# xiaolong-li1/VIDEO-BLADE

Measured on AMD Instinct MI355X. Metric: frames/sec (aggregate over n_gpus; per GPU = value/n_gpus), CogVideoX-5B 8-step 49x720x480 bf16 (attention path); attn TFLOPS vs dense, higher is better.
Workload: dtype bf16; 1 GPU; CogVideoX-5B 8-step 49x720x480 bf16: 336 inner_attention calls per video (8 steps x 42 blocks), q/k/v [1,48,17776,64] (13x30x45 latent tokens + 226 text); global_batch=1, seq_len=17776, heads=48, head_dim=64, mask=energy rule (reference defaults), parallelism=replicas x1 (prompt-batch DP, no collective)

## Files before the change

video-blade_amd/csrc/vb_attn_fwd.hip:

```cpp
#include <type_traits>

#include "vb_args.hpp"
#include "vb_attn_fwd.hpp"
#include "vb_trace.hpp"

#ifndef VB_ATTN_TRACE
#define VB_ATTN_TRACE 0
#endif
#if VB_ATTN_TRACE
namespace vb { __device__ TraceBuf g_attn_trace; }
#define VB_ATRACE_START(k) trace_start(g_attn_trace, k, (unsigned)vblk)
#define VB_ATRACE_END() trace_end(g_attn_trace, (unsigned)vblk)
#else
#define VB_ATRACE_START(k)
#define VB_ATRACE_END()
#endif

namespace vb {

#ifndef VB_LAZY_COUNT
#define VB_LAZY_COUNT 0
#endif
#if VB_LAZY_COUNT
__device__ unsigned long long g_vb_stamp[16];
#define VB_LAZY_ADD(slot, n) if (lane == 0) atomicAdd(&g_vb_stamp[slot], n)
#else
#define VB_LAZY_ADD(slot, n)
#endif

template <int D, bool kKvRows>
constexpr int fwd_smem_bytes() {
  return ((D == 64) ? 3 : 2) * 2 * kKT * D * 2 + kMaxBlocks * 2 + 16 + (kKvRows ? 4 * 512 : 0);
}

__device__ __forceinline__ int ballot_rank(unsigned long long bal) {
  return __builtin_amdgcn_mbcnt_hi((unsigned)(bal >> 32), __builtin_amdgcn_mbcnt_lo((unsigned)bal, 0u));
}
__device__ __forceinline__ void build_kept_list(const uint8_t* mrow, bool dense, bool use_main, int nbk, int qblk,
                                                int lane, uint16_t* list, int* list_n) {
  int n = 0;
  int dpos = -1;
  if (use_main) {
    for (int j0 = 0; j0 < nbk; j0 += 64) {
      const int j = j0 + lane;
      const bool keep = (j < nbk) && (dense || mrow[j] != 0);
      const unsigned long long bal = __ballot(keep);
      if (keep) {
        const int pos = n + ballot_rank(bal);
        list[pos] = (uint16_t)j;
        if (j == qblk) dpos = pos;
      }
      n += __popcll(bal);
    }
    const unsigned long long db = __ballot(dpos > 0);
    if (db != 0 && qblk != nbk - 1) {
      const int dp = __builtin_amdgcn_readlane(dpos, (int)__builtin_ctzll(db));
      if (lane == 0) {
        const uint16_t t = list[0];
        list[0] = (uint16_t)qblk;
        list[dp] = t;
      }
    }
  }
  if (lane == 0) *list_n = n;
}

__device__ __forceinline__ float half_max(const f32x16& x) {
  const float a = max3f(max3f(max3f(x[0], x[1], x[2]), x[3], x[4]), x[5], x[6]);
  const float c = max3f(max3f(max3f(x[8], x[9], x[10]), x[11], x[12]), x[13], x[14]);
  return max3f(a, c, fmaxf(x[7], x[15]));
}
template <class T, int kPrio>
__device__ __forceinline__ float exp_pack(const f32x16& x, typename T::vec8& p0, typename T::vec8& p1) {
  float e[16];
  float h4[4];
  if constexpr (kPrio & 4) __builtin_amdgcn_s_setprio(1);
#pragma unroll
  for (int r = 0; r < 16; ++r) {
    e[r] = exp2_fast(x[r]);
    h4[r & 3] = r < 4 ? e[r] : h4[r & 3] + e[r];
  }
  u32x4 u0, u1;
#pragma unroll
  for (int w = 0; w < 4; ++w) {
    u0[w] = pack2<T>(e[2 * w], e[2 * w + 1]);
    u1[w] = pack2<T>(e[8 + 2 * w], e[8 + 2 * w + 1]);
  }
  p0 = __builtin_bit_cast(typename T::vec8, u0);
  p1 = __builtin_bit_cast(typename T::vec8, u1);
  if constexpr (kPrio & 4) __builtin_amdgcn_s_setprio(0);
  return (h4[0] + h4[1]) + (h4[2] + h4[3]);
}


template <int D, class T, bool kPool, bool kKvRows, bool kML, bool kCBias, bool kWQ>
__device__ __forceinline__ void attn_fwd_item(const FwdParams& p, const int vblk, int& next) {
  constexpr int KS = D / 16;
  constexpr int DT = D / 32;
  constexpr bool kSplitPV = fwd::split_pv(D);
  constexpr int kPrio = !kCBias ? 0 : D == 64 ? fwd::kPrio64 : fwd::kPrio128;
  constexpr float kLazyBound = std::is_same<T, BF16>::value ? kLazyBoundBF16 : kLazyBoundF16;
  constexpr int kRowB = D * 2;
  constexpr int kMatBytes = kKT * kRowB;
  constexpr int kBufBytes = 2 * kMatBytes;
  constexpr int kBufs = (D == 64) ? 3 : 2;
  constexpr int kChunks = kRowB / 16;
  constexpr int kRowsPerInst = 1024 / kRowB;
  constexpr int kInstPerMat = kMatBytes / 1024;
  constexpr int kInstPerWave = 2 * kInstPerMat / 4;
  __shared__ __attribute__((aligned(16))) uint8_t smem[fwd_smem_bytes<D, kKvRows>()];
  static_assert(fwd_smem_bytes<D, kKvRows>() == kBufs * kBufBytes + kMaxBlocks * 2 + 16 + (kKvRows ? 4 * 512 : 0), "LDS layout");
  static_assert(!(kML && (kPool || kKvRows)), "multi-level mode reads the KV pyramids only");
  uint16_t* list = reinterpret_cast<uint16_t*>(smem + kBufs * kBufBytes);
  int* list_n = reinterpret_cast<int*>(smem + kBufs * kBufBytes + kMaxBlocks * 2);

  int tid = threadIdx.x;
  if constexpr (kWQ) {
    asm volatile("" : "+v"(tid));
    tid &= kThreads - 1;
  }
  const int lane = tid & 63;
  const int wave = __builtin_amdgcn_readfirstlane(tid >> 6);

  const int half = lane >> 5;
  const int l32 = lane & 31;

  VB_ATRACE_START(0);
  int qblk, bh;
  fwd_item_decode(p, vblk, bh, qblk);
  const int b = bh / p.H, h = bh % p.H;

  int Lq = p.Lq, Lk = p.Lk;
  int64_t qrow0 = 0, krow0 = 0;
  if (p.cu_q) {
    qrow0 = p.cu_q[b];
    Lq = p.cu_q[b + 1] - p.cu_q[b];
    krow0 = p.cu_k[b];
    Lk = p.cu_k[b + 1] - p.cu_k[b];
  }
  const int q0 = qblk * kQBlk;
  if (q0 >= Lq) return;
  const int nbk = (Lk + kQBlk - 1) / kQBlk;

  const uint8_t* mrow = nullptr;
  bool dense = true;
  bool nan_head = false;
  if (p.use_main) {
    const uint8_t* mh = head_mask_base(p.mask, p.ms, p.head_mask_type, p.H, b, h, nan_head, p.hm_mode);
    if (mh) {
      dense = false;
      mrow = mh + (int64_t)qblk * p.ms[2];
    }
  }
  if (kML) {
    if (tid < 64) {
      int cnt[4] = {0, 0, 0, 0};
      for (int j0 = 0; j0 < nbk; j0 += 64) {
        const int j = j0 + lane;
        const int lv = j < nbk ? mrow[j] : 0;
#pragma unroll
        for (int e = 0; e < 4; ++e) cnt[e] += __popcll(__ballot(lv == (1 << e)));
      }
      int pos[4] = {0, cnt[0], cnt[0] + cnt[1], cnt[0] + cnt[1] + cnt[2]};
      for (int j0 = 0; j0 < nbk; j0 += 64) {
        const int j = j0 + lane;
        const int lv = j < nbk ? mrow[j] : 0;
#pragma unroll
        for (int e = 0; e < 4; ++e) {
          const unsigned long long bal = __ballot(lv == (1 << e));
          if (lv == (1 << e))
            list[pos[e] + __builtin_amdgcn_mbcnt_hi((unsigned)(bal >> 32),
                                                    __builtin_amdgcn_mbcnt_lo((unsigned)bal, 0u))] = (uint16_t)j;
          pos[e] += __popcll(bal);
        }
      }
      if (lane < 4) list_n[lane] = cnt[0] * (lane == 0) + cnt[1] * (lane == 1) + cnt[2] * (lane == 2) + cnt[3] * (lane == 3);
    }
  } else if (tid < 64) {
    build_kept_list(mrow, dense, p.use_main, nbk, qblk, lane, list, list_n);
  }

  const int qg = q0 + wave * 32 + l32;
  const bool qvalid = qg < Lq;
  int qrow = qvalid ? qg : Lq - 1;
  if (p.q_rows) qrow = p.q_rows[qrow];
  const uint8_t* qbase = reinterpret_cast<const uint8_t*>(p.q) + 2 * (b * p.qs[0] + h * p.qs[1] + qrow0 * p.qs[2]);
  typename T::vec8 qf[KS];
  auto load_q = [&]() __attribute__((always_inline)) {
    const uint8_t* qp = qbase + (int64_t)qrow * 2 * p.qs[2];
#pragma unroll
    for (int s = 0; s < KS; ++s)
      qf[s] = *reinterpret_cast<const typename T::vec8*>(qp + (16 * s + 8 * half) * 2);
    if constexpr (kCBias) {
#pragma unroll
      for (int s = 0; s < KS; ++s)
#pragma unroll
        for (int e = 0; e < 8; ++e) qf[s][e] = T::from_f32(T::to_f32(qf[s][e]) * p.c);
    }
#pragma unroll
    for (int s = 0; s < KS; ++s) asm volatile("" : "+v"(qf[s]));
  };
  constexpr bool kQLate = D == 64 ? fwd::kQLate64 : (kCBias && !kKvRows) ? fwd::kQLate128Lazy : fwd::kQLate128;
  if constexpr (kQLate) {
    asm volatile("s_waitcnt lgkmcnt(0)" ::: "memory");
    __builtin_amdgcn_s_barrier();
    asm volatile("" ::: "memory");
  } else {
    load_q();
    __syncthreads();
  }
  const int nkept = __builtin_amdgcn_readfirstlane(*list_n);
  int ntm = 2 * nkept;
  if (nkept > 0 && list[nkept - 1] == nbk - 1 && (nbk - 1) * kQBlk + kKT >= Lk && !(kML && p.ref_tail)) ntm -= 1;
  const int ntp = kPool ? (p.Lkp + kKT - 1) / kKT : 0;
  int n2 = 0, n4 = 0, n8 = 0, T12 = 0, T124 = 0;
  if (kML) {
    n2 = __builtin_amdgcn_readfirstlane(list_n[1]);
    n4 = __builtin_amdgcn_readfirstlane(list_n[2]);
    n8 = __builtin_amdgcn_readfirstlane(list_n[3]);
    T12 = ntm + n2;
    T124 = T12 + (n4 + 1) / 2;
  }
  const int ntiles = kML ? T124 + (n8 + 3) / 4 : ntm + ntp;

  const uint8_t* kbase = reinterpret_cast<const uint8_t*>(p.k) + 2 * (b * p.ks[0] + h * p.ks[1] + krow0 * p.ks[2]);
  const uint8_t* vbase = reinterpret_cast<const uint8_t*>(p.v) + 2 * (b * p.vs[0] + h * p.vs[1] + krow0 * p.vs[2]);
  const uint8_t* kpbase = nullptr;
  const uint8_t* vpbase = nullptr;
  if (kPool) {
    kpbase = reinterpret_cast<const uint8_t*>(p.kp) + 2 * (b * p.kps[0] + h * p.kps[1]);
    vpbase = reinterpret_cast<const uint8_t*>(p.vp) + 2 * (b * p.vps[0] + h * p.vps[1]);
  }

  auto tile_src = [&](int t, int blk_raw) __attribute__((always_inline)) -> TileSrc {
    TileSrc s;
    if (t < ntm) {
      const int blk = __builtin_amdgcn_readfirstlane(blk_raw);
      s.pooled = 0;
      s.kstart = blk * kQBlk + (t & 1) * kKT;
      s.klen = min(kKT, Lk - s.kstart);
    } else {
      s.pooled = 1;
      s.kstart = (t - ntm) * kKT;
      s.klen = min(kKT, p.Lkp - s.kstart);
    }
    return s;
  };

  const int off4 = p.Lpad + p.Lpad / 2, off8 = off4 + p.Lpad / 4;
  const int my_half = (wave & 1) * 32;
  auto ml_tile_src = [&](int t, int raw) __attribute__((always_inline)) -> MlTileSrc {
    MlTileSrc s;
    const int a = __builtin_amdgcn_readfirstlane(raw & 0xFFFF);
    const int c = __builtin_amdgcn_readfirstlane(raw >> 16);
    if (t < ntm) {
      const int kstart = a * kQBlk + (t & 1) * kKT;
      s.srcA = kstart + my_half;
      s.klen = p.ref_tail ? kKT : min(kKT, Lk - kstart);
      s.lvl = 0;
    } else if (t < T12) {
      s.srcA = p.Lpad + a * 64 + my_half;
      s.klen = kKT;
      s.lvl = 1;
    } else if (t < T124) {
      s.srcA = off4 + a * 32;
      s.klen = min(kKT, (n4 - 2 * (t - T12)) * 32);
      s.lvl = 2;
    } else {
      s.srcA = off8 + a * 16;
      s.klen = min(kKT, (n8 - 4 * (t - T124)) * 16);
      s.lvl = 3;
    }
    s.srcB = (t >= T124) ? off8 + c * 16 : s.srcA + 16;
    return s;
  };
  auto ml_list_at = [&](int t) __attribute__((always_inline)) -> int {
    int e0, e1;
    if (t < ntm) {
      e0 = e1 = t >> 1;
    } else if (t < T12) {
      e0 = e1 = nkept + (t - ntm);
    } else if (t < T124) {
      e0 = e1 = nkept + n2 + min(2 * (t - T12) + (wave & 1), n4 - 1);
    } else {
      const int e = 4 * (t - T124) + 2 * (wave & 1);
      e0 = nkept + n2 + n4 + min(e, n8 - 1);
      e1 = nkept + n2 + n4 + min(e + 1, n8 - 1);
    }
    e0 = min(max(e0, 0), kMaxBlocks - 1);
    e1 = min(max(e1, 0), kMaxBlocks - 1);
    return (int)list[e0] | ((int)list[e1] << 16);
  };

  static_assert(2 * kInstPerWave == kInstPerMat, "DMA split assumes two waves per matrix");
  const int my_mat = wave >> 1;
  const uint8_t* my_base = my_mat == 0 ? kbase : vbase;
  const int64_t my_stride = 2 * (my_mat == 0 ? p.ks[2] : p.vs[2]);
  const uint8_t* my_pbase = my_mat == 0 ? kpbase : vpbase;
  const int64_t my_pstride = kPool ? 2 * (my_mat == 0 ? p.kps[2] : p.vps[2]) : 0;
  int my_chunk[kInstPerWave];
  int my_row[kInstPerWave];
#pragma unroll
  for (int i = 0; i < kInstPerWave; ++i) {
    const int mi = (wave & 1) * kInstPerWave + i;
    const int r = mi * kRowsPerInst + lane / kChunks;
    const int sl = lane % kChunks;
    my_row[i] = r;
    if (my_mat == 0) {
      my_chunk[i] = sl ^ ((D == 64) ? ((r >> 1) & 7) : (r & 15));
    } else {
      const int vsw = (D == 64) ? ((r >> 1) & 1) : (r & 3);
      my_chunk[i] = (((sl >> 2) ^ vsw) << 2) | (sl & 3);
    }
  }
  const int my_rowb = (int)my_stride;
  const int my_prowb = (int)my_pstride;
  const int src_rows = kML ? 15 * (p.Lpad / 8) : Lk;
  const srd_t my_rsrc = make_srd(my_base, p.use_main ? (int)((int64_t)(src_rows - 1) * my_stride + kRowB) : 0);
  const srd_t my_prsrc = make_srd(kPool ? my_pbase : my_base, kPool ? (int)((int64_t)(p.Lkp - 1) * my_pstride + kRowB) : 0);
  int my_voff[kInstPerWave];
  int my_rc[kInstPerWave];
  const int my_row0 = my_row[0];
#pragma unroll
  for (int i = 0; i < kInstPerWave; ++i) {
    my_rc[i] = my_chunk[i] * 16;
    if constexpr (kML) my_voff[i] = (my_row[i] & 15) * my_rowb + my_chunk[i] * 16;
  }
  auto ml_issue = [&](const MlTileSrc src, int slot) __attribute__((always_inline)) {
    uint8_t* dst = smem + slot * kBufBytes + my_mat * kMatBytes + (wave & 1) * kInstPerWave * 1024;
    const int soffA = __builtin_amdgcn_readfirstlane(src.srcA * my_rowb);
    const int soffB = __builtin_amdgcn_readfirstlane(src.srcB * my_rowb);
#pragma unroll
    for (int i = 0; i < kInstPerWave; ++i)
      if constexpr (kWQ) dma16_unscoped(my_rsrc, dst + i * 1024, my_voff[i], (i * kRowsPerInst >= 16) ? soffB : soffA);
      else dma16(my_rsrc, dst + i * 1024, my_voff[i], (i * kRowsPerInst >= 16) ? soffB : soffA);
  };
  const int gather_key = ((wave & 1) * kInstPerWave + (lane % kInstPerWave)) * kRowsPerInst + lane / kInstPerWave;
  const srd_t rows_srd = make_srd(kKvRows ? p.kv_rows : nullptr, kKvRows ? Lk * 4 : 0);
  uint8_t* const ibase = smem + kBufs * kBufBytes + kMaxBlocks * 2 + 16 + wave * 128;
  auto issue_idx = [&](int t, int blk_raw) __attribute__((always_inline)) {
    int voff = 0;
    if (t < ntm) {
      const int kstart = __builtin_amdgcn_readfirstlane(blk_raw) * kQBlk + (t & 1) * kKT;
      voff = 4 * (kstart + min(gather_key, min(kKT, Lk - kstart) - 1));
    }
    if (lane < 32) {
      uint8_t* dst = ibase + (t & 3) * 512;
      if constexpr (kWQ) {
        uint32_t a = __builtin_amdgcn_readfirstlane(
            static_cast<uint32_t>(reinterpret_cast<uintptr_t>((__attribute__((address_space(3))) uint8_t*)dst)));
        asm("" : "+s"(a));
        dst = (uint8_t*)(__attribute__((address_space(3))) uint8_t*)(uintptr_t)a;
      }
      __builtin_amdgcn_raw_ptr_buffer_load_lds(
          __builtin_amdgcn_make_buffer_rsrc(const_cast<void*>(rows_srd.base), (short)0, rows_srd.bytes, 0x00020000),
          (__attribute__((address_space(3))) void*)dst, 4, voff, 0, 0, 0);
    }
  };
  auto issue = [&](const TileSrc src, int slot, int t = 0) __attribute__((always_inline)) {
    uint8_t* dst = smem + slot * kBufBytes + my_mat * kMatBytes + (wave & 1) * kInstPerWave * 1024;
    auto piece = [&](int i, srd_t sd, int voff, int soff) __attribute__((always_inline)) {
      if constexpr (kWQ) dma16_unscoped(sd, dst + i * 1024, voff, soff);
      else dma16(sd, dst + i * 1024, voff, soff);
    };
    const bool pooled = kPool && src.pooled;
    if (kKvRows && !pooled) {
      typedef int i32x4 __attribute__((ext_vector_type(4)));
      int o[kInstPerWave];
      const uint8_t* ib = ibase + (t & 3) * 512 + 4 * kInstPerWave * (lane / kChunks);
#pragma unroll
      for (int c = 0; c < kInstPerWave; c += 4) {
        const i32x4 w = *reinterpret_cast<const i32x4*>(ib + 4 * c);
#pragma unroll
        for (int e = 0; e < 4; ++e) o[c + e] = w[e];
      }
#pragma unroll
      for (int i = 0; i < kInstPerWave; ++i) {
        int voff;
        asm("v_mad_u32_u24 %0, %1, %2, %3" : "=v"(voff) : "v"(o[i]), "s"(my_rowb), "v"(my_chunk[i] * 16));
        piece(i, my_rsrc, voff, 0);
      }
      return;
    }
    const int rowb = pooled ? my_prowb : my_rowb;
    const int soff = __builtin_amdgcn_readfirstlane(src.kstart * rowb);
    if (src.klen == kKT) {
      const int vb0 = (int)__umul24((unsigned)my_row0, (unsigned)rowb);
#pragma unroll
      for (int i = 0; i < kInstPerWave; ++i)
        piece(i, pooled ? my_prsrc : my_rsrc, vb0 + my_rc[i], __builtin_amdgcn_readfirstlane(soff + i * kRowsPerInst * rowb));
    } else {
#pragma unroll
      for (int i = 0; i < kInstPerWave; ++i) {
        const int r = min(my_row0 + i * kRowsPerInst, src.klen - 1);
        piece(i, pooled ? my_prsrc : my_rsrc, r * rowb + my_rc[i], soff);
      }
    }
  };

  f32x16 o[DT];
#pragma unroll
  for (int i = 0; i < DT; ++i)
#pragma unroll
    for (int r = 0; r < 16; ++r) o[i][r] = 0.f;
  float m = kCBias ? 0.f : -INFINITY;
  float l = 0.f;
  f32x16 cb;
#pragma unroll
  for (int r = 0; r < 16; ++r) cb[r] = 0.f;
  int cur_bias_bits = 0;
  bool first = true;

  const int vrow = 4 * half + (lane & 15) / 4;
  const int vcol = 16 * ((lane >> 4) & 1) + 4 * (lane & 3);

  int k_lane[KS];
#pragma unroll
  for (int ks = 0; ks < KS; ++ks) k_lane[ks] = k_off<D>(l32, 2 * ks + half);
  uint32_t v_lane[DT];
#pragma unroll
  for (int dt = 0; dt < DT; ++dt)
    v_lane[dt] = static_cast<uint32_t>(reinterpret_cast<uintptr_t>(
                     (__attribute__((address_space(3))) const uint8_t*)smem)) +
                 v_off_bytes<D>(vrow, dt * 32 + vcol);

  auto tile_step = [&](auto U, int bias_bits, int klen) __attribute__((always_inline)) {
    constexpr int kSlot = decltype(U)::value;
    const uint8_t* kl = smem + kSlot * kBufBytes;
    const float bias = __int_as_float(bias_bits);
    f32x16 s[2];
    constexpr int VPRE = D == 64 ? (kKvRows ? fwd::kVPre64Rows : fwd::kVPre64) : 2;
    s16x4 vlo[4][DT], vhi[4][DT];
    auto read_v = [&](int kk) __attribute__((always_inline)) {
      const int row0 = (kk >> 1) * 32 + 16 * (kk & 1);
#pragma unroll
      for (int dt = 0; dt < DT; ++dt) {
        vlo[kk][dt] = lds_tr4_asm(v_lane[dt], kSlot * kBufBytes + kMatBytes + row0 * kRowB);
        vhi[kk][dt] = lds_tr4_asm(v_lane[dt], kSlot * kBufBytes + kMatBytes + (row0 + 8) * kRowB);
      }
    };
    auto wait_v = [&](int kk) __attribute__((always_inline)) {
#pragma unroll
      for (int dt = 0; dt < DT; ++dt)
        asm volatile("s_waitcnt lgkmcnt(0)" : "+v"(vlo[kk][dt]), "+v"(vhi[kk][dt]));
    };
    auto next_v = [&](int kk) __attribute__((always_inline)) {
      wait_v(kk);
      if (kk + VPRE < 4) read_v(kk + VPRE);
    };
    auto pv = [&](int kk, const typename T::vec8& pf) __attribute__((always_inline)) {
      if constexpr (kPrio & 2) __builtin_amdgcn_s_setprio(1);
#pragma unroll
      for (int dt = 0; dt < DT; ++dt) o[dt] = T::mfma32(join8<T>(vlo[kk][dt], vhi[kk][dt]), pf, o[dt]);
      if constexpr (kPrio & 2) __builtin_amdgcn_s_setprio(0);
    };
    auto mask_tail = [&](int kt) __attribute__((always_inline)) {
#pragma unroll
      for (int r = 0; r < 16; ++r)
        if (kt * 32 + (r & 3) + 8 * (r >> 2) + 4 * half >= klen) s[kt][r] = -INFINITY;
    };
    auto scores = [&](const f32x16& seed) __attribute__((always_inline)) {
      if constexpr (kPrio & 1) __builtin_amdgcn_s_setprio(1);
#pragma unroll
      for (int kt = 0; kt < 2; ++kt) {
        typename T::vec8 kf[KS];
#pragma unroll
        for (int ks = 0; ks < KS; ++ks) kf[ks] = lds_b128<T>(kl + kt * 32 * kRowB, k_lane[ks]);
        s[kt] = T::mfma32(kf[0], qf[0], seed);
#pragma unroll
        for (int ks = 1; ks < KS; ++ks) s[kt] = T::mfma32(kf[ks], qf[ks], s[kt]);
      }
      if constexpr (kPrio & 1) __builtin_amdgcn_s_setprio(0);
    };

    if constexpr (kCBias) {
      if (bias_bits != cur_bias_bits) {
        asm volatile("");
        const float db = bias - __int_as_float(cur_bias_bits);
#pragma unroll
        for (int r = 0; r < 16; ++r) cb[r] += db;
        cur_bias_bits = bias_bits;
      }
      auto raise_m = [&](float mt, auto KT0) __attribute__((always_inline)) {
        constexpr int kt0 = decltype(KT0)::value;
        const float delta = fmaxf(max_xor32(mt), 0.f);
        const float alpha = exp2_fast(-delta);
        m += delta;
        l *= alpha;
#pragma unroll
        for (int i = 0; i < DT; ++i)
#pragma unroll
          for (int r = 0; r < 16; ++r) o[i][r] *= alpha;
#pragma unroll
        for (int r = 0; r < 16; ++r) {
          cb[r] -= delta;
          if (kt0 == 0) s[0][r] -= delta;
          s[1][r] -= delta;
        }
      };
      scores(cb);
#pragma unroll
      for (int kk = 0; kk < VPRE; ++kk) read_v(kk);
      if (klen < kKT) {
        asm volatile("");
        mask_tail(0);
        mask_tail(1);
      }
      if (first) {
        asm volatile("");
        const float mt = max_xor32(fmaxf(half_max(s[0]), half_max(s[1])));
        m += mt;
#pragma unroll
        for (int r = 0; r < 16; ++r) {
          s[0][r] -= mt;
          s[1][r] -= mt;
          cb[r] -= mt;
        }
        first = false;
      }
      typename T::vec8 pf[4];
      if constexpr (kSplitPV) {
#pragma unroll
        for (int kt = 0; kt < 2; ++kt) {
          float hs = exp_pack<T, kPrio>(s[kt], pf[2 * kt], pf[2 * kt + 1]);
          if (!__all(hs <= kLazyBound)) {
            asm volatile("");
            VB_LAZY_ADD(10, 1ull);
            if (kt == 0) raise_m(half_max(s[0]), std::integral_constant<int, 0>{});
            else raise_m(half_max(s[1]), std::integral_constant<int, 1>{});
            hs = exp_pack<T, kPrio>(s[kt], pf[2 * kt], pf[2 * kt + 1]);
          }
          l += hs;
#pragma unroll
          for (int kk = 2 * kt; kk < 2 * kt + 2; ++kk) {
            next_v(kk);
            pv(kk, pf[kk]);
          }
        }
      } else {
        float h0 = exp_pack<T, kPrio>(s[0], pf[0], pf[1]);
        float h1 = exp_pack<T, kPrio>(s[1], pf[2], pf[3]);
        if (!__all(fmaxf(h0, h1) <= kLazyBound)) {
          asm volatile("");
          VB_LAZY_ADD(10, 1ull);
          raise_m(fmaxf(half_max(s[0]), half_max(s[1])), std::integral_constant<int, 0>{});
          h0 = exp_pack<T, kPrio>(s[0], pf[0], pf[1]);
          h1 = exp_pack<T, kPrio>(s[1], pf[2], pf[3]);
        }
        l += h0 + h1;
#pragma unroll
        for (int kk = 0; kk < 4; ++kk) {
          next_v(kk);
          pv(kk, pf[kk]);
        }
      }
      VB_LAZY_ADD(11, kSplitPV ? 2ull : 1ull);
    }

    if constexpr (!kCBias) {
      f32x16 zero;
#pragma unroll
      for (int r = 0; r < 16; ++r) zero[r] = 0.f;
      scores(zero);
#pragma unroll
      for (int kk = 0; kk < VPRE; ++kk) read_v(kk);
      if (klen < kKT) {
        asm volatile("");
#pragma unroll
        for (int kt = 0; kt < 2; ++kt)
#pragma unroll
          for (int r = 0; r < 16; ++r)
            if (kt * 32 + (r & 3) + 8 * (r >> 2) + 4 * half >= klen) s[kt][r] = -INFINITY;
      }
      float mq[4];
#pragma unroll
      for (int c = 0; c < 4; ++c) {
        const f32x16& x = s[c >> 1];
        const int o = 8 * (c & 1);
        mq[c] = max3f(max3f(max3f(x[o], x[o + 1], x[o + 2]), x[o + 3], x[o + 4]), x[o + 5], x[o + 6]);
      }
      const float f1 = max3f(mq[0], mq[1], s[0][7]);
      const float f2 = max3f(mq[2], mq[3], s[0][15]);
      float mt = max3f(max3f(f1, f2, s[1][7]), s[1][15], s[1][15]);
      mt = max_xor32(mt) * p.c + bias;
      if (!__all(mt <= m + fwd::kRescaleSlack)) {
        asm volatile("");
        const float mn = fmaxf(m, mt);
        const float alpha = exp2_fast(m - mn);
        m = mn;
        l *= alpha;
#pragma unroll
        for (int i = 0; i < DT; ++i)
#pragma unroll
          for (int r = 0; r < 16; ++r) o[i][r] *= alpha;
      }
      const float nbias = bias - m;
      float lq[4] = {0.f, 0.f, 0.f, 0.f};
      if constexpr (kSplitPV) {
#pragma unroll
        for (int kt = 0; kt < 2; ++kt) {
#pragma unroll
          for (int r = 0; r < 16; ++r) {
            const float e = exp2_fast(fmaf(s[kt][r], p.c, nbias));
            s[kt][r] = e;
            lq[(2 * kt + r) & 3] = (kt == 0 && r < 4) ? e : lq[(2 * kt + r) & 3] + e;
          }
#pragma unroll
          for (int kk = 2 * kt; kk < 2 * kt + 2; ++kk) {
            wait_v(kk);
            if (kk + VPRE < 4) read_v(kk + VPRE);
            const typename T::vec8 pf = pack8<T>(s[kk >> 1], 8 * (kk & 1));
#pragma unroll
            for (int dt = 0; dt < DT; ++dt) o[dt] = T::mfma32(join8<T>(vlo[kk][dt], vhi[kk][dt]), pf, o[dt]);
          }
        }
        l += (lq[0] + lq[1]) + (lq[2] + lq[3]);
      } else {
#pragma unroll
        for (int kt = 0; kt < 2; ++kt)
#pragma unroll
          for (int r = 0; r < 16; ++r) {
            const float e = exp2_fast(fmaf(s[kt][r], p.c, nbias));
            s[kt][r] = e;
            lq[(2 * kt + r) & 3] = (kt == 0 && r < 4) ? e : lq[(2 * kt + r) & 3] + e;
          }
        l += (lq[0] + lq[1]) + (lq[2] + lq[3]);
#pragma unroll
        for (int kk = 0; kk < 4; ++kk) {
          wait_v(kk);
          if (kk + VPRE < 4) read_v(kk + VPRE);
          const typename T::vec8 pf = pack8<T>(s[kk >> 1], 8 * (kk & 1));
#pragma unroll
          for (int dt = 0; dt < DT; ++dt) o[dt] = T::mfma32(join8<T>(vlo[kk][dt], vhi[kk][dt]), pf, o[dt]);
        }
      }
    }
  };

  auto list_at = [&](int t) __attribute__((always_inline)) -> int {
    return t < ntm ? (int)list[min(t >> 1, kMaxBlocks - 1)] : 0;
  };
  using Src = std::conditional_t<kML, MlTileSrc, TileSrc>;
  auto any_list_at = [&](int t) __attribute__((always_inline)) -> int {
    if constexpr (kML) return ml_list_at(t);
    else return list_at(t);
  };
  auto any_tile_src = [&](int t, int raw) __attribute__((always_inline)) -> Src {
    if constexpr (kML) return ml_tile_src(t, raw);
    else return tile_src(t, raw);
  };
  auto any_issue = [&](const Src src, int slot) __attribute__((always_inline)) {
    if constexpr (kML) ml_issue(src, slot);
    else issue(src, slot);
  };
  Src slot_src[kBufs];
  const int pool_bias_bits = __builtin_amdgcn_readfirstlane(__float_as_int(p.pool_bias_l2));
  int next_blk, idx_blk = 0;
  if constexpr (kKvRows) {
#pragma unroll
    for (int s0 = 0; s0 < kBufs; ++s0) issue_idx(s0, list_at(s0));
    slot_src[0] = tile_src(0, list_at(0));
    VB_WAIT_VMCNT(kBufs - 1);
    asm volatile("" ::: "memory");
    issue(slot_src[0], 0, 0);
    if constexpr (kBufs > 2) {
      slot_src[1] = tile_src(1, list_at(1));
      VB_WAIT_VMCNT(kBufs - 2 + kInstPerWave);
      asm volatile("" ::: "memory");
      issue(slot_src[1], 1, 1);
    }
    next_blk = list_at(kBufs - 1);
    idx_blk = list_at(kBufs);
  } else {
    slot_src[0] = any_tile_src(0, any_list_at(0));
    if (ntiles > 0) any_issue(slot_src[0], 0);
    if constexpr (kBufs > 2) {
      slot_src[1] = any_tile_src(1, any_list_at(1));
      if (ntiles > 1) any_issue(slot_src[1], 1);
    }
    next_blk = any_list_at(kBufs - 1);
  }
  if constexpr (kQLate) load_q();
  auto body = [&](int t, auto U) __attribute__((always_inline)) {
    constexpr int u = decltype(U)::value;
    constexpr int un = (u + kBufs - 1) % kBufs;
    const int ti = t + kBufs - 1;
    if constexpr (kKvRows) {
      if constexpr (kBufs == 3) VB_WAIT_VMCNT(kInstPerWave);
      else VB_WAIT_VMCNT(0);
      asm volatile("s_waitcnt lgkmcnt(0)" ::: "memory");
      __builtin_amdgcn_s_barrier();
      asm volatile("" ::: "memory");
      issue_idx(t + kBufs, idx_blk);
      slot_src[un] = tile_src(ti, next_blk);
      issue(slot_src[un], un, ti);
      next_blk = idx_blk;
      idx_blk = list_at(t + kBufs + 1);
    } else {
      const int younger = min(ntiles - 1 - t, kBufs - 2);
      if (younger >= 2) VB_WAIT_VMCNT(2 * kInstPerWave);
      else if (younger == 1) VB_WAIT_VMCNT(kInstPerWave);
      else VB_WAIT_VMCNT(0);
      asm volatile("s_waitcnt lgkmcnt(0)" ::: "memory");
      __builtin_amdgcn_s_barrier();
      if (ti < ntiles) {
        slot_src[un] = any_tile_src(ti, next_blk);
        any_issue(slot_src[un], un);
        next_blk = any_list_at(ti + 1);
      }
    }
    const Src src = slot_src[u];
    int bias_bits;
    if constexpr (kML) {
      bias_bits = src.lvl == 0 ? 0 : src.lvl == 1 ? 0x3F800000 : src.lvl == 2 ? 0x40000000 : 0x40400000;
    } else {
      bias_bits = (kPool && src.pooled) ? pool_bias_bits : 0;
    }
    bias_bits = __builtin_amdgcn_readfirstlane(bias_bits);
    tile_step(U, bias_bits, src.klen);
  };
  for (int t0 = 0; t0 < ntiles; t0 += kBufs) {
    body(t0, std::integral_constant<int, 0>{});
    if (t0 + 1 < ntiles) body(t0 + 1, std::integral_constant<int, 1>{});
    if constexpr (kBufs > 2)
      if (t0 + 2 < ntiles) body(t0 + 2, std::integral_constant<int, 2>{});
  }
  if constexpr (kKvRows || kWQ) VB_WAIT_VMCNT(0);
  if (kWQ && tid == 0) next = wq_fetch(p.work_queue, blockIdx.x & 7, p.n_items);

  const float lt = add_xor32(l);
  const float inv = (lt > 0.f) ? 1.0f / lt : 0.f;
  constexpr uint32_t kNaN2 = std::is_same<T, BF16>::value ? 0x7FC07FC0u : 0x7E007E00u;
  if (qvalid) {
    uint8_t* obase = reinterpret_cast<uint8_t*>(p.out) +
                     2 * (b * p.os[0] + h * p.os[1] + (qrow0 + qrow) * p.os[2]);
#pragma unroll
    for (int dt = 0; dt < DT; ++dt)
#pragma unroll
      for (int pr = 0; pr < 2; ++pr) {
        u32x2 a, c;
        a[0] = pack2<T>(o[dt][8 * pr + 0] * inv, o[dt][8 * pr + 1] * inv);
        a[1] = pack2<T>(o[dt][8 * pr + 2] * inv, o[dt][8 * pr + 3] * inv);
        c[0] = pack2<T>(o[dt][8 * pr + 4] * inv, o[dt][8 * pr + 5] * inv);
        c[1] = pack2<T>(o[dt][8 * pr + 6] * inv, o[dt][8 * pr + 7] * inv);
        if (nan_head) a[0] = a[1] = c[0] = c[1] = kNaN2;
        const auto sx = __builtin_amdgcn_permlane32_swap(a[0], c[0], false, false);
        const auto sy = __builtin_amdgcn_permlane32_swap(a[1], c[1], false, false);
        const u32x4 w = {sx[0], sy[0], sx[1], sy[1]};
        *reinterpret_cast<u32x4*>(obase + (dt * 32 + 16 * pr + 8 * half) * 2) = w;
      }
    if (p.lse && half == 0) {
      const float v = (m + __log2f(lt)) * kLn2;
      float* dst = p.lse + b * p.lse_s[0] + h * p.lse_s[1] + (p.cu_q ? qg : qrow);
      if (nan_head) *reinterpret_cast<uint32_t*>(dst) = 0x7FC00000u;
      else *dst = (p.cu_q && !(lt > 0.f)) ? INFINITY : v;
    }
  }
  VB_ATRACE_END();
}

template <int D, class T, bool kPool, bool kKvRows, bool kML = false, bool kCBias = false, bool kPersist = false>
__global__ void __launch_bounds__(kThreads, (D == 64 ? fwd::kWavesD64 : 2)) attn_fwd_kernel(const FwdParams p) {
  if constexpr (!kPersist) {
    int next;
    attn_fwd_item<D, T, kPool, kKvRows, kML, kCBias, false>(p, blockIdx.x, next);
  } else {
    __shared__ int next_s;
    int* const wq = p.work_queue;
    if (threadIdx.x == 0) next_s = wq_fetch(wq, blockIdx.x & 7, p.n_items);
    __syncthreads();
    int item = next_s;
    while (item >= 0) {
      int next = -2;
      attn_fwd_item<D, T, kPool, kKvRows, kML, kCBias, true>(p, item, next);
      if (threadIdx.x == 0) next_s = next == -2 ? wq_fetch(wq, blockIdx.x & 7, p.n_items) : next;
      __syncthreads();
      item = next_s;
      __syncthreads();
    }
    if (threadIdx.x == 0) wq_finish(wq);
  }
}

constexpr int kOrderBins = 8192;
__global__ void __launch_bounds__(1024) attn_order_kernel(const FwdParams p, int32_t* order) {
  __shared__ int bins[kOrderBins];
  const int BH = p.B * p.H;
  const int hr = min(p.heavy_rows, p.nbq);
  const int rows_left = p.nbq - hr;
  const int nwg = rows_left * BH;
  const int x = blockIdx.x;
  const int q8 = nwg >> 3, r8 = nwg & 7;
  int start = x < r8 ? x * (q8 + 1) : r8 * (q8 + 1) + (x - r8) * q8;
  const int count_x = q8 + (x < r8 ? 1 : 0);
  if (count_x <= 0) return;
  const int skip = (p.order_window > 0 && p.order_window < count_x) ? count_x - p.order_window : 0;
  for (int i = threadIdx.x; i < skip; i += blockDim.x) order[start + i] = start + i;
  start += skip;
  const int count = count_x - skip;
  const int bh0 = start / rows_left;
  const int nh = (start + count - 1) / rows_left - bh0 + 1;
  const int nl = p.nbk + 1;
  const bool by_head = (int64_t)nh * nl <= kOrderBins;
  const int nbins = by_head ? nh * nl : nl;
  for (int i = threadIdx.x; i < nbins; i += blockDim.x) bins[i] = 0;
  __syncthreads();
  auto key_of = [&](int lin) -> int {
    int bh, qblk;
    fwd_phase2_item(lin, rows_left, bh, qblk);
    bool nan_head = false;
    const uint8_t* mh = head_mask_base(p.mask, p.ms, p.head_mask_type, p.H, bh / p.H, bh % p.H, nan_head, p.hm_mode);
    int kept = p.nbk;
    if (p.q_len) {
      kept = min(max(p.q_len[(int64_t)bh * p.nbq + qblk], 0), p.nbk);
    } else if (mh) {
      const uint8_t* mrow = mh + (int64_t)qblk * p.ms[2];
      kept = 0;
      for (int j = 0; j < p.nbk; ++j) kept += mrow[j] != 0;
    }
    return (by_head ? (bh - bh0) * nl : 0) + (p.nbk - kept);
  };
  for (int i = threadIdx.x; i < count; i += blockDim.x) atomicAdd(&bins[key_of(start + i)], 1);
  __syncthreads();
  {
    __shared__ int wsum[16];
    const int C = (nbins + 1023) / 1024;
    const int b0 = threadIdx.x * C;
    int run = 0;
    for (int i = 0; i < C; ++i) run += (b0 + i < nbins) ? bins[b0 + i] : 0;
    const int lane = threadIdx.x & 63, w = threadIdx.x >> 6;
    int incl = run;
    for (int o = 1; o < 64; o <<= 1) {
      const int y = __shfl_up(incl, o);
      if (lane >= o) incl += y;
    }
    if (lane == 63) wsum[w] = incl;
    __syncthreads();
    int wbase = 0;
    for (int i = 0; i < w; ++i) wbase += wsum[i];
    int pos = wbase + incl - run;
    for (int i = 0; i < C; ++i) {
      if (b0 + i < nbins) {
        const int c = bins[b0 + i];
        bins[b0 + i] = pos;
        pos += c;
      }
    }
  }
  __syncthreads();
  for (int i = threadIdx.x; i < count; i += blockDim.x) {
    const int lin = start + i;
    order[start + atomicAdd(&bins[key_of(lin)], 1)] = lin;
  }
}

template <auto Kern, auto KernP>
static int launch_one(FwdParams p, hipStream_t stream, const char* what) {
  const unsigned items = (unsigned)(p.nbq * p.B * p.H);
  p.n_items = (int)items;
  if (p.work_queue) {
    const unsigned slots = (unsigned)resident_grid(reinterpret_cast<const void*>(KernP), kThreads, 0);
    hipLaunchKernelGGL(KernP, dim3(slots < items ? slots : items), dim3(kThreads), 0, stream, p);
  } else {
    hipLaunchKernelGGL(Kern, dim3(items), dim3(kThreads), 0, stream, p);
  }
  return check_launch(what);
}

template <int D, class T, bool kPool, bool kKvRows, bool kML, bool kCBias>
static int launch_attn(const FwdParams& p, hipStream_t stream, const char* what) {
  return launch_one<attn_fwd_kernel<D, T, kPool, kKvRows, kML, kCBias, false>,
                    attn_fwd_kernel<D, T, kPool, kKvRows, kML, kCBias, true>>(p, stream, what);
}

int launch_fwd(const FwdParams& p, int D, int dtype, bool pool, hipStream_t stream) {
  return dispatch_head(D, dtype, [&](auto d, auto t, auto pl, auto rows, auto cb) {
    return launch_attn<d(), decltype(t), pl(), rows(), false, cb()>(p, stream, "attn_fwd_kernel");
  }, pool, p.kv_rows != nullptr, p.lse == nullptr);
}

int launch_ml_fwd(const FwdParams& p, int D, int dtype, hipStream_t stream) {
  return dispatch_head(D, dtype, [&](auto d, auto t, auto cb) {
    return launch_attn<d(), decltype(t), false, false, true, cb()>(p, stream, "attn_fwd_kernel (multi-level)");
  }, p.lse == nullptr);
}

int launch_attn_order(const FwdParams& p, int32_t* order, hipStream_t stream) {
  hipLaunchKernelGGL(attn_order_kernel, dim3(8), dim3(1024), 0, stream, p, order);
  return check_launch("attn_order_kernel");
}

}

#if VB_LAZY_COUNT
extern "C" int vb_diag_stamps(unsigned long long* host16, int reset) {
  (void)hipDeviceSynchronize();
  (void)hipMemcpyFromSymbol(host16, HIP_SYMBOL(vb::g_vb_stamp), sizeof(unsigned long long) * 16);
  if (reset) {
    unsigned long long z[16] = {0};
    (void)hipMemcpyToSymbol(HIP_SYMBOL(vb::g_vb_stamp), z, sizeof(z));
  }
  return 0;
}
#endif

#if VB_ATTN_TRACE
VB_TRACE_GETTER(vb_debug_attn_trace, vb::g_attn_trace)
#endif
```

video-blade_amd/csrc/vb_attn_fwd.hpp:

```cpp
#pragma once
#include "vb_tiles.hpp"

namespace vb {

struct FwdParams {
  const void* q; const void* k; const void* v;
  int64_t qs[3], ks[3], vs[3];
  const int32_t* q_rows; const int32_t* kv_rows;
  const int32_t* cu_q; const int32_t* cu_k;
  const int32_t* head_mask_type;
  int hm_mode;
  int use_main;
  const uint8_t* mask; int64_t ms[3];
  const void* kp; const void* vp; int64_t kps[3], vps[3];
  int Lkp; float pool_bias_l2;
  void* out; int64_t os[3];
  float* lse; int64_t lse_s[2];
  int B, H, Lq, Lk, nbq, nbk;
  float c;
  int heavy_rows;
  const int32_t* q_order;
  const int32_t* q_len;
  int order_window;
  int Lpad;
  int ref_tail;
  int* work_queue;
  int n_items;
};

constexpr int kThreads = 256;
constexpr int kQBlk = 128;
constexpr int kKT = 64;
constexpr int kMaxBlocks = 1024;

namespace fwd {
constexpr int kVPre64 = 4;
constexpr int kVPre64Rows = 3;
constexpr bool split_pv(int D) { return D == 64; }
constexpr int kPrio64 = 0;
constexpr int kPrio128 = 3;
constexpr bool kQLate64 = true;
constexpr bool kQLate128 = true;
constexpr bool kQLate128Lazy = false;
constexpr int kWavesD64 = 3;
constexpr float kRescaleSlack = 4.0f;
}
constexpr float kLazyBoundBF16 = 4294967296.0f;
constexpr float kLazyBoundF16 = 256.0f;

template <int D>
__device__ __forceinline__ int k_off(int row, int ch) {
  constexpr int kRowBytes = D * 2;
  const int sw = (D == 64) ? ((row >> 1) & 7) : (row & 15);
  return row * kRowBytes + 16 * (ch ^ sw);
}
template <int D>
__device__ __forceinline__ int v_off_bytes(int row, int col) {
  constexpr int kRowBytes = D * 2;
  const int g = col >> 5;
  const int sw = (D == 64) ? ((row >> 1) & 1) : (row & 3);
  return row * kRowBytes + 64 * (g ^ sw) + (col & 31) * 2;
}

struct TileSrc {
  int pooled;
  int kstart;
  int klen;
};

struct MlTileSrc {
  int srcA, srcB;
  int klen;
  int lvl;
};

__device__ __forceinline__ void fwd_phase2_item(int lin, int rows_left, int& bh, int& qblk) {
  bh = lin / rows_left;
  qblk = rows_left - 1 - lin % rows_left;
}
__device__ __forceinline__ void fwd_item_decode(const FwdParams& p, int vblk, int& bh, int& qblk) {
  const int BH = p.B * p.H;
  const int hr = min(p.heavy_rows, p.nbq);
  const int n_heavy = hr * BH;
  if (vblk < n_heavy) {
    qblk = p.nbq - 1 - vblk / BH;
    bh = vblk % BH;
  } else {
    const int rows_left = p.nbq - hr;
    int lin = xcd_linear(vblk - n_heavy, rows_left * BH);
    if (p.q_order) lin = __builtin_amdgcn_readfirstlane(p.q_order[lin]);
    fwd_phase2_item(lin, rows_left, bh, qblk);
  }
}

int launch_fwd(const FwdParams& p, int D, int dtype, bool pool, hipStream_t stream);
int launch_ml_fwd(const FwdParams& p, int D, int dtype, hipStream_t stream);
int launch_attn_order(const FwdParams& p, int32_t* order, hipStream_t stream);

}
```

Measured before the change: 146.2 frames/s.

## Peel first KV tile and overlap second-half QK MFMAs with first-half exp for D=64

For head_dim 64 with the pooled bias path, the first KV tile is peeled out of the loop so the running-max initialisation no longer needs a per-tile branch. Steady-state tiles interleave the MFMAs for the second 32-row score half with exp2/pack of the first half, and issue V-transpose LDS reads between them using sched_barriers. The aim is to hide transcendental latency under matrix-core work. In exchange, tail tiles recompute exp after masking, register pressure rises, and the loop ring order is rotated to start at slot 1.

```diff
diff --git a/video-blade_amd/csrc/vb_attn_fwd.hip b/video-blade_amd/csrc/vb_attn_fwd.hip
--- a/video-blade_amd/csrc/vb_attn_fwd.hip
+++ b/video-blade_amd/csrc/vb_attn_fwd.hip
@@ -424,7 +424,7 @@
                      (__attribute__((address_space(3))) const uint8_t*)smem)) +
                  v_off_bytes<D>(vrow, dt * 32 + vcol);
 
-  auto tile_step = [&](auto U, int bias_bits, int klen) __attribute__((always_inline)) {
+  auto tile_step = [&](auto U, auto MODE, int bias_bits, int klen) __attribute__((always_inline)) {
     constexpr int kSlot = decltype(U)::value;
     const uint8_t* kl = smem + kSlot * kBufBytes;
     const float bias = __int_as_float(bias_bits);
@@ -498,31 +498,82 @@
           s[1][r] -= delta;
         }
       };
-      scores(cb);
-#pragma unroll
-      for (int kk = 0; kk < VPRE; ++kk) read_v(kk);
-      if (klen < kKT) {
-        asm volatile("");
-        mask_tail(0);
-        mask_tail(1);
-      }
-      if (first) {
-        asm volatile("");
-        const float mt = max_xor32(fmaxf(half_max(s[0]), half_max(s[1])));
-        m += mt;
-#pragma unroll
-        for (int r = 0; r < 16; ++r) {
-          s[0][r] -= mt;
-          s[1][r] -= mt;
-          cb[r] -= mt;
+      if constexpr (D == 64) {
+        constexpr int kMode = decltype(MODE)::value;
+        constexpr bool kOverlap = kMode == fwd::kTileSteady && fwd::s_under_exp64(kPool, kKvRows, kML, kWQ);
+        typename T::vec8 pf[4];
+        float hs;
+        if constexpr (kOverlap) {
+          static_assert(VPRE == 4 && KS == 4, "the placed tile reads all four V^T k-steps ahead");
+          typename T::vec8 kf0[KS], kf1[KS];
+#pragma unroll
+          for (int ks = 0; ks < KS; ++ks) kf0[ks] = lds_b128<T>(kl, k_lane[ks]);
+          kf1[0] = lds_b128<T>(kl + 32 * kRowB, k_lane[0]);
+          kf1[1] = lds_b128<T>(kl + 32 * kRowB, k_lane[1]);
+          s[0] = T::mfma32(kf0[0], qf[0], cb);
+#pragma unroll
+          for (int ks = 1; ks < KS; ++ks) s[0] = T::mfma32(kf0[ks], qf[ks], s[0]);
+          s[1] = T::mfma32(kf1[0], qf[0], cb);
+          float e[16], h4[4];
+          u32x4 u0, u1;
+          auto exp_part = [&](int r0, int r1) __attribute__((always_inline)) {
+#pragma unroll
+            for (int r = r0; r < r1; ++r) {
+              e[r] = exp2_fast(s[0][r]);
+              h4[r & 3] = r < 4 ? e[r] : h4[r & 3] + e[r];
+              if (r & 1) (r < 8 ? u0 : u1)[(r & 7) >> 1] = pack2<T>(e[r - 1], e[r]);
+            }
+          };
+          __builtin_amdgcn_sched_barrier(0);
+          kf1[2] = lds_b128<T>(kl + 32 * kRowB, k_lane[2]);
+          kf1[3] = lds_b128<T>(kl + 32 * kRowB, k_lane[3]);
+          read_v(0);
+          read_v(1);
+          __builtin_amdgcn_sched_barrier(0);
+#pragma unroll
+          for (int ks = 1; ks < KS; ++ks) {
+            exp_part((ks - 1) * fwd::kExpPerMfma64, ks * fwd::kExpPerMfma64);
+            __builtin_amdgcn_sched_barrier(0);
+            s[1] = T::mfma32(kf1[ks], qf[ks], s[1]);
+            __builtin_amdgcn_sched_barrier(0);
+          }
+          exp_part((KS - 1) * fwd::kExpPerMfma64, 16);
+          read_v(2);
+          read_v(3);
+          pf[0] = __builtin_bit_cast(typename T::vec8, u0);
+          pf[1] = __builtin_bit_cast(typename T::vec8, u1);
+          hs = (h4[0] + h4[1]) + (h4[2] + h4[3]);
+          if (klen < kKT) {
+            asm volatile("");
+            mask_tail(0);
+            mask_tail(1);
+            hs = exp_pack<T, kPrio>(s[0], pf[0], pf[1]);
+          }
+        } else {
+          scores(cb);
+#pragma unroll
+          for (int kk = 0; kk < VPRE; ++kk) read_v(kk);
+          if (klen < kKT) {
+            asm volatile("");
+            mask_tail(0);
+            mask_tail(1);
+          }
+          if constexpr (kMode == fwd::kTilePeel) {
+            const float mt = max_xor32(fmaxf(half_max(s[0]), half_max(s[1])));
+            m += mt;
+#pragma unroll
+            for (int r = 0; r < 16; ++r) {
+              s[0][r] -= mt;
+              s[1][r] -= mt;
+              cb[r] -= mt;
+            }
+          }
+          hs = exp_pack<T, kPrio>(s[0], pf[0], pf[1]);
         }
-        first = false;
-      }
-      typename T::vec8 pf[4];
-      if constexpr (kSplitPV) {
+        static_assert(kSplitPV, "the D=64 tile splits P.V");
 #pragma unroll
         for (int kt = 0; kt < 2; ++kt) {
-          float hs = exp_pack<T, kPrio>(s[kt], pf[2 * kt], pf[2 * kt + 1]);
+          if (kt == 1) hs = exp_pack<T, kPrio>(s[1], pf[2], pf[3]);
           if (!__all(hs <= kLazyBound)) {
             asm volatile("");
             VB_LAZY_ADD(10, 1ull);
@@ -538,6 +589,28 @@
           }
         }
       } else {
+        static_assert(!kSplitPV, "the D=128 tile keeps P.V whole");
+        scores(cb);
+#pragma unroll
+        for (int kk = 0; kk < VPRE; ++kk) read_v(kk);
+        if (klen < kKT) {
+          asm volatile("");
+          mask_tail(0);
+          mask_tail(1);
+        }
+        if (first) {
+          asm volatile("");
+          const float mt = max_xor32(fmaxf(half_max(s[0]), half_max(s[1])));
+          m += mt;
+#pragma unroll
+          for (int r = 0; r < 16; ++r) {
+            s[0][r] -= mt;
+            s[1][r] -= mt;
+            cb[r] -= mt;
+          }
+          first = false;
+        }
+        typename T::vec8 pf[4];
         float h0 = exp_pack<T, kPrio>(s[0], pf[0], pf[1]);
         float h1 = exp_pack<T, kPrio>(s[1], pf[2], pf[3]);
         if (!__all(fmaxf(h0, h1) <= kLazyBound)) {
@@ -681,7 +754,8 @@
     next_blk = any_list_at(kBufs - 1);
   }
   if constexpr (kQLate) load_q();
-  auto body = [&](int t, auto U) __attribute__((always_inline)) {
+  constexpr bool kTile64 = D == 64 && kCBias;
+  auto body = [&](int t, auto U, auto PEEL) __attribute__((always_inline)) {
     constexpr int u = decltype(U)::value;
     constexpr int un = (u + kBufs - 1) % kBufs;
     const int ti = t + kBufs - 1;
@@ -717,13 +791,24 @@
       bias_bits = (kPool && src.pooled) ? pool_bias_bits : 0;
     }
     bias_bits = __builtin_amdgcn_readfirstlane(bias_bits);
-    tile_step(U, bias_bits, src.klen);
-  };
-  for (int t0 = 0; t0 < ntiles; t0 += kBufs) {
-    body(t0, std::integral_constant<int, 0>{});
-    if (t0 + 1 < ntiles) body(t0 + 1, std::integral_constant<int, 1>{});
-    if constexpr (kBufs > 2)
-      if (t0 + 2 < ntiles) body(t0 + 2, std::integral_constant<int, 2>{});
+    constexpr int kMode = (kTile64 && decltype(PEEL)::value) ? fwd::kTilePeel : fwd::kTileSteady;
+    tile_step(U, std::integral_constant<int, kMode>{}, bias_bits, src.klen);
+  };
+  if constexpr (kTile64) {
+    static_assert(kBufs == 3, "the peeled loop walks a 3-slot ring");
+    if (ntiles > 0) body(0, std::integral_constant<int, 0>{}, std::true_type{});
+    for (int t0 = 1; t0 < ntiles; t0 += kBufs) {
+      body(t0, std::integral_constant<int, 1>{}, std::false_type{});
+      if (t0 + 1 < ntiles) body(t0 + 1, std::integral_constant<int, 2>{}, std::false_type{});
+      if (t0 + 2 < ntiles) body(t0 + 2, std::integral_constant<int, 0>{}, std::false_type{});
+    }
+  } else {
+    for (int t0 = 0; t0 < ntiles; t0 += kBufs) {
+      body(t0, std::integral_constant<int, 0>{}, std::false_type{});
+      if (t0 + 1 < ntiles) body(t0 + 1, std::integral_constant<int, 1>{}, std::false_type{});
+      if constexpr (kBufs > 2)
+        if (t0 + 2 < ntiles) body(t0 + 2, std::integral_constant<int, 2>{}, std::false_type{});
+    }
   }
   if constexpr (kKvRows || kWQ) VB_WAIT_VMCNT(0);
   if (kWQ && tid == 0) next = wq_fetch(p.work_queue, blockIdx.x & 7, p.n_items);
diff --git a/video-blade_amd/csrc/vb_attn_fwd.hpp b/video-blade_amd/csrc/vb_attn_fwd.hpp
--- a/video-blade_amd/csrc/vb_attn_fwd.hpp
+++ b/video-blade_amd/csrc/vb_attn_fwd.hpp
@@ -43,6 +43,9 @@
 constexpr bool kQLate128 = true;
 constexpr bool kQLate128Lazy = false;
 constexpr int kWavesD64 = 3;
+enum { kTileSteady = 0, kTilePeel = 1 };
+constexpr bool s_under_exp64(bool pool, bool kv_rows, bool ml, bool wq) { return pool && !kv_rows && !ml && !wq; }
+constexpr int kExpPerMfma64 = 4;
 constexpr float kRescaleSlack = 4.0f;
 }
 constexpr float kLazyBoundBF16 = 4294967296.0f;
```

Result: no change. 146.4 frames/s, median of 6 (+0.1%).
